# treangenlab/komb

Hardware: AMD Instinct MI355X
Metric: peeled edges/sec (k-truss) (higher is better)
Workload: dtype int32

## Files before the change

### include/komb_accel.h

```cpp
#ifndef KOMB_ACCEL_H
#define KOMB_ACCEL_H

#include <stdint.h>

#ifdef __cplusplus
extern "C" {
#endif

#define KOMB_ACCEL_ABI_VERSION 7

typedef enum komb_status {
    KOMB_OK          =  0,
    KOMB_ERR_ARG     = -1,
    KOMB_ERR_DEVICE  = -2,
    KOMB_ERR_NOMEM   = -3,
    KOMB_ERR_LIMIT   = -4,
    KOMB_ERR_STATE   = -5
} komb_status;

typedef struct komb_ctx komb_ctx;

typedef struct komb_opts {
    int32_t device;
    int32_t verbosity;
// ... 22 lines not shown
    double  ms_compact;
    double  ms_support;
    double  ms_allreduce;
    double  ms_peel;
    double  ms_gather;
    double  ms_corea;
    double  ms_tail;
    int64_t core_local_items, truss_local_items;
    int32_t core_local_units, core_local_sweeps;
    int32_t truss_local_units, truss_local_sweeps;
    double  ms_core_local;
    double  ms_truss_local;
    double  ms_sort;
    int64_t tri_records;
    int32_t index_layout;
    int32_t shard_exchanges;
    double  ms_exchange;
    int64_t exchange_words;
    double  ms_build_h2d;
    double  ms_build_relabel;
    double  ms_prepare;
    int32_t truss_prepared;
    int32_t engine_flags;
    double  ms_prep_vertex;
    double  ms_prep_edges;
    double  ms_prep_rows;
    int32_t stream_retries;
    int32_t reserved0;
} komb_stats;
#define KOMB_ENGINE_LOCAL_FINISH 1
#define KOMB_ENGINE_LDS_TAIL     2
#define KOMB_ENGINE_SHARD_PEEL   4
#define KOMB_ENGINE_TWO_PASS     8

komb_ctx   *komb_create(const komb_opts *opts);
void        komb_destroy(komb_ctx *ctx);
const char *komb_last_error(const komb_ctx *ctx);
int         komb_abi_version(void);
int         komb_set_option(komb_ctx *ctx, const char *name, const char *value);

int komb_graph_from_edges(komb_ctx *ctx, int64_t nv, int64_t n_raw,
                          const int64_t *uv_pairs);

int komb_graph_from_csr(komb_ctx *ctx, int64_t nv, const int64_t *rowptr,
                        const int32_t *col);

int komb_graph_info(komb_ctx *ctx, int64_t *nv, int64_t *ne);

int komb_graph_get_csr(komb_ctx *ctx, int64_t *rowptr, int32_t *col);

int komb_core_run(komb_ctx *ctx);
typedef int (*komb_allreduce_fn)(void *user, void *device_u32, int64_t count);
int komb_core_run_sharded(komb_ctx *ctx, int32_t rank, int32_t world, komb_allreduce_fn allreduce, void *user);
int komb_core_fetch(komb_ctx *ctx, int32_t *degree , int32_t *coreness );
int komb_degree_coreness(komb_ctx *ctx, int32_t *degree, int32_t *coreness);

int komb_onion_run(komb_ctx *ctx);
int komb_onion_fetch(komb_ctx *ctx, int32_t *layer , int32_t *coreness );
int komb_onion_info(komb_ctx *ctx, int64_t *n_layers, int32_t *max_coreness, double *ms);

#define KOMB_COMP_CORE   0
#define KOMB_COMP_TRUSS  1
#define KOMB_COMP_K_MAX (-1)
int komb_components_run(komb_ctx *ctx, int32_t kind, int32_t k);
int komb_components_fetch(komb_ctx *ctx, int32_t *label , int32_t *size );
int komb_components_info(komb_ctx *ctx, int32_t *kind, int32_t *k_used, int64_t *n_members,
// ... 34 lines not shown
```

### komb_amd/api.py

```python
import ctypes
import os

import numpy as np

from . import _lib
from ._lib import KombOpts, KombStats, as_c, ptr


class KombError(RuntimeError):
    def __init__(self, code, msg):
        super().__init__(f"komb_accel error {code}: {msg}")
        self.code = code


def gen_hug_edges(nv, n_cliques, alpha=2.6, seed=42):
    lib = _lib.load()
    n_raw = lib.komb_gen_hug_edges(nv, n_cliques, alpha, seed, None)
    if n_raw < 0:
        raise ValueError("komb_gen_hug_edges: bad arguments")
    uv = np.empty((n_raw, 2), dtype=np.int64)
    got = lib.komb_gen_hug_edges(nv, n_cliques, alpha, seed, ptr(uv))
    assert got == n_raw
    return uv


FORWARD_ENV_OPTIONS = False
OPTION_NAMES = ("FINISH", "LOCAL_LIMIT", "LOCAL_ITEMS", "LOCAL_DENSITY", "LOCAL_DEFER_CHUNKS", "TAIL", "CORE_TAIL", "INDEX",
                "REC_CAP", "OWN_DENSE_CAP", "NO_OWN_DENSE", "NO_REC_SCRATCH", "NO_FIRST_QUEUE", "FULL_CAPS", "PREP_ROW_STAGE", "RETIRE_EVERY", "SHARD_ENGINE",
                "TRI_DEBUG", "POOL_DEBUG", "BUILD_DEBUG", "LOCAL_DEBUG", "TAIL_DEBUG", "COMP_SAMPLE", "POISON")

SENTINEL_I32 = -0x5A5A5A5B


def _out_i32(n):
    return np.full(n, SENTINEL_I32, dtype=np.int32)


def _out_f64(n):
    return np.full(n, np.nan, dtype=np.float64)


class KombAccel:
    def __init__(self, device=0, verbosity=0, flags=0):
        self._lib = _lib.load()
        opts = KombOpts(device=device, verbosity=verbosity)
        opts.reserved[0] = flags
        self._ctx = self._lib.komb_create(ctypes.byref(opts))
        if not self._ctx:
            raise MemoryError("komb_create failed")
        self.device = device
        self.nv = -1
        self.ne = 0
        self._forwarded = {}

    def set_option(self, name, value):
        v = None if value is None else str(value).encode()
        self._check(self._lib.komb_set_option(self._ctx, name.encode(), v))

    def _sync_env_options(self):
        if not FORWARD_ENV_OPTIONS:
            return
# ... 193 lines not shown
```

### komb_amd/csrc/api.cpp

```cpp
#include "common.h"

#include <cerrno>
#include <cmath>
#include <cstdlib>
#include <cstring>
#include <memory>
#include <new>
#include <vector>

using namespace komb;

namespace {

int require_device(komb_ctx *ctx)
{
    if (!ctx) return KOMB_ERR_ARG;
    if (!ctx->device_ok) {
        if (ctx->err.empty()) ctx->err = "no usable HIP device";
        return KOMB_ERR_DEVICE;
    }
    KOMB_HIP(ctx, hipSetDevice(ctx->device));
    ctx->err.clear();
    return KOMB_OK;
}

}

extern "C" {

int komb_abi_version(void) { return KOMB_ACCEL_ABI_VERSION; }

komb_ctx *komb_create(const komb_opts *opts)
{
    komb_ctx *ctx = new (std::nothrow) komb_ctx();
    if (!ctx) return nullptr;
    if (opts) ctx->opts = *opts;
    ctx->device = ctx->opts.device;
    int ndev = 0;
    hipError_t e = hipGetDeviceCount(&ndev);
    if (e != hipSuccess || ndev <= 0) {
        ctx->err = std::string("no usable HIP device: ") + (e != hipSuccess ? hipGetErrorString(e) : "device count is 0");
        (void)hipGetLastError();
        return ctx;
    }
    if (ctx->device < 0 || ctx->device >= ndev) {
        ctx->err = "device ordinal out of range";
        return ctx;
    }
    e = hipSetDevice(ctx->device);
    if (e == hipSuccess) e = hipHostMalloc((void **)&ctx->h_ctrl, 2 * sizeof(PeelCtrl), hipHostMallocDefault);
    if (e == hipSuccess) e = hipHostMalloc((void **)&ctx->h_local, 2 * sizeof(LocalCtrl), hipHostMallocDefault);
    if (e == hipSuccess) e = hipHostMalloc(&ctx->h_stage, kStageBytes, hipHostMallocDefault);
    ctx->stream = nullptr;
    if (e == hipSuccess && !(ctx->opts.reserved[0] & KOMB_CREATE_NULL_STREAM)) { e = hipStreamCreate(&ctx->stream); ctx->own_stream = e == hipSuccess; }
    if (e == hipSuccess && !ctx->timer.init()) e = hipErrorUnknown;
    if (e != hipSuccess) {
        ctx->err = std::string("device initialisation failed: ") + hipGetErrorString(e);
        return ctx;
    }
    ctx->device_ok = true;
    if (!(ctx->opts.reserved[0] & KOMB_CREATE_NO_WARMUP)) warm_up(ctx);
    return ctx;
}

void komb_destroy(komb_ctx *ctx)
{
    if (!ctx) return;
    if (ctx->device_ok) {
        (void)hipSetDevice(ctx->device);
        graph_free(ctx);
        stager_free(ctx);
        ctx->pool.clear();
        ctx->timer.destroy();
        if (ctx->own_stream && ctx->stream) (void)hipStreamDestroy(ctx->stream);
        if (ctx->h_ctrl) (void)hipHostFree(ctx->h_ctrl);
        if (ctx->h_local) (void)hipHostFree(ctx->h_local);
        if (ctx->h_stage) (void)hipHostFree(ctx->h_stage);
    }
    delete ctx;
}

const char *komb_last_error(const komb_ctx *ctx) { return ctx ? ctx->err.c_str() : "null context"; }

int komb_graph_from_edges(komb_ctx *ctx, int64_t nv, int64_t n_raw, const int64_t *uv_pairs)
{
    KOMB_TRY(require_device(ctx));
    return graph_from_edges(ctx, nv, n_raw, uv_pairs);
}

int komb_graph_from_csr(komb_ctx *ctx, int64_t nv, const int64_t *rowptr, const int32_t *col)
{
    KOMB_TRY(require_device(ctx));
    return graph_from_csr(ctx, nv, rowptr, col);
}

int komb_graph_info(komb_ctx *ctx, int64_t *nv, int64_t *ne)
{
    if (!ctx) return KOMB_ERR_ARG;
    if (ctx->nv < 0) KOMB_FAIL(ctx, KOMB_ERR_STATE, "komb_graph_info: no graph loaded");
    if (nv) *nv = ctx->nv;
    if (ne) *ne = ctx->ne;
    return KOMB_OK;
}

int komb_graph_get_csr(komb_ctx *ctx, int64_t *rowptr, int32_t *col)
{
// ... 264 lines not shown
```

### komb_amd/csrc/common.h

```cpp
#pragma once

#include <hip/hip_runtime.h>

#include <chrono>
#include <cstddef>
#include <cstdint>
#include <cstdio>
#include <cstdlib>
#include <cstring>
#include <map>
#include <string>
#include <vector>

#include "komb_accel.h"

#include <roctracer/roctx.h>

namespace komb {

struct Range {
    explicit Range(const char *name) { (void)roctxRangePushA(name); }
    ~Range() { (void)roctxRangePop(); }
    void next(const char *name) { (void)roctxRangePop(); (void)roctxRangePushA(name); }
    Range(const Range &) = delete;
// ... 159 lines not shown
        for (auto &b : blocks) { if (b.used) keep.push_back(b); else (void)hipFree(b.p); }
        blocks.swap(keep);
    }
    void clear()
    {
        for (auto &b : blocks) (void)hipFree(b.p);
        blocks.clear();
    }
};

struct TrussPrep {
    bool valid = false;
    int64_t nv = 0, ne = 0;
    int32_t  *o2i = nullptr, *i2o = nullptr;
    uint32_t *orow = nullptr;
    int32_t  *ocol = nullptr, *osrc = nullptr;
    uint32_t *e2k = nullptr;
    uint4    *vline = nullptr;
    void     *wtasks = nullptr;
    int64_t   n_wtasks = 0;
    int64_t   own_bound = 0;
    double    ms = 0.0;
    double    ms_part[4] = {0, 0, 0, 0};
};

struct komb_ctx {
    komb_opts opts{};
    DevPool pool;
    std::string err;
    bool device_ok = false;
    int device = 0;
    hipStream_t stream = nullptr;
    bool own_stream = false;
    komb::Timer timer;
    std::map<std::string, std::string> options;

    int64_t nv = -1, ne = 0;
    uint32_t *d_o_rowptr = nullptr;
    int32_t  *d_o_col = nullptr;
    TrussPrep prep;

    int32_t *d_deg = nullptr;
    int32_t *d_core = nullptr;
    bool core_done = false;

    int32_t *d_onion_layer = nullptr;
    int32_t *d_onion_core = nullptr;
    int64_t onion_layers = 0;
    int32_t onion_max_core = 0;
    double onion_ms = 0.0;
    bool onion_done = false;

    int32_t *d_comp_label = nullptr;
    int32_t *d_comp_size = nullptr;
    int32_t comp_kind = 0, comp_k = 0;
    int64_t comp_members = 0, comp_count = 0, comp_largest = 0;
    double comp_ms = 0.0;
    bool comp_done = false;

    int64_t t_ne = -1;
    int32_t *d_t_eu = nullptr, *d_t_ev = nullptr, *d_t_truss = nullptr, *d_t_sup = nullptr;
    uint2 *d_t_slice = nullptr;
    uint32_t t_k_lo = 0, t_k_hi = 0;
    bool t_sup_ready = false;
    bool t_own_edges = false;
    int32_t *d_ceu = nullptr, *d_cev = nullptr;
// ... 241 lines not shown
```

### komb_amd/csrc/kcore.hip

```cpp
#include "peel_dev.h"
#include "core_tail.h"
#include "local_dev.h"
#include "shard_dev.h"

#include <cstdlib>

namespace komb {

namespace {

__global__ __launch_bounds__(kBlock) void k_core_init(const uint32_t *__restrict__ rowptr, int64_t nv,
                                                      int32_t *__restrict__ deg, int32_t *__restrict__ degw,
                                                      int32_t *__restrict__ core, uint32_t *__restrict__ init)
{
    uint32_t zeros = 0;
    int32_t lmin = 0x7FFFFFFF;
    for (int64_t v = (int64_t)blockIdx.x * kBlock + threadIdx.x; v < nv; v += (int64_t)gridDim.x * kBlock) {
        const int32_t d = (int32_t)(rowptr[v + 1] - rowptr[v]);
        deg[v] = d; degw[v] = d;
        if (d == 0) { core[v] = 0; ++zeros; }
        else { core[v] = alive_marker((uint32_t)d); lmin = min(lmin, d); }
    }
    block_add_min(zeros, lmin, &init[0], (int32_t *)&init[1]);
}
// ... 242 lines not shown
    peel_ctrl_pre(s, d_grp);
    k_core_init<<<grid_init, kBlock, 0, s>>>(ctx->d_o_rowptr, nv, ctx->d_deg, d_degw, ctx->d_core, d_grp + kInitOff);
    peel_ctrl_init(s, d_ctrl, d_grp, (uint32_t)nv, tail_limit);
    auto run_tail = [&](const int32_t *list, uint32_t n_in) -> int {
        KOMB_HIP(ctx, hipMemsetAsync(T.livebits, 0, live_words * sizeof(unsigned long long), s));
        KOMB_HIP(ctx, hipMemsetAsync(T.cnt, 0, 4 * sizeof(uint32_t), s));
        KOMB_HIP(ctx, hipMemsetAsync(T.rows, 0, (size_t)kCoreTailV * kCoreTailWords * sizeof(unsigned long long), s));
        int64_t gm = ((int64_t)n_in + kBlock - 1) / kBlock;
        k_ctail_mark<<<(int)(gm < 1 ? 1 : (gm > 1024 ? 1024 : gm)), kBlock, 0, s>>>(list, n_in, ctx->d_core, T);
        k_ctail_rows<<<dim3(kCoreTailV, 8), kBlock, 0, s>>>(ctx->d_o_rowptr, ctx->d_o_col, T);
        k_core_tail<false><<<1, 1024, 0, s>>>(d_ctrl, T, d_degw, ctx->d_core, nullptr);
        KOMB_HIP(ctx, d2h(ctx, &ctx->h_ctrl[0], d_ctrl, sizeof(PeelCtrl)));
        return KOMB_OK;
    };
    auto run_local = [&]() -> int {
        const PeelCtrl hc = ctx->h_ctrl[0];
        Range r_local("core: local finish");
        EventSet evs;
        hipEvent_t ev[2] = {nullptr, nullptr};
        for (auto &e : ev) KOMB_HIP(ctx, evs.make(&e));
        (void)hipEventRecord(ev[0], s);
        KOMB_HIP(ctx, hipMemsetAsync(d_livebits, 0, live_words * sizeof(unsigned long long), s));
        LocalStats ls;
        const int rc = local_finish(ctx, bufs, hc, d_ctrl, (uint32_t)nv, ctx->d_core, d_degw, Q.live[hc.live_sel],
            (uint32_t)kWave * CoreLocal::kU, sizeof(uint32_t), local_item_limit(ctx, std::max<uint64_t>(kCoreLocalItems, (uint64_t)ctx->ne / 3)), 0u, false, 0, ctx->d_core,
            [&](const LocalGraph &lg, const int32_t *num, void *items, PeelCtrl *d_cctrl, int32_t launch) {
                CoreCollect C{(uint32_t)nv, ctx->d_o_rowptr, ctx->d_o_col, ctx->d_core, d_livebits, num, lg.off, lg.cur, (uint32_t *)items};
                k_peel_step<CoreCollect><<<grid, kPeelBlock, 0, s>>>(d_cctrl, d_grp, Q, C, launch);
            },
            [&](const LocalGraph &lg, void *items, uint64_t total, LocalCtrl *d_lctrl, uint32_t *d_cnt, int *launches) -> int {
                return local_fixpoint(ctx, d_lctrl, d_cnt, lg, CoreLocal{(const uint32_t *)items}, total, launches);
            },
            &ls,
            [&](const LocalGraph &lg) { k_live_bits<<<(int)((lg.n + 255) / 256 > 1024 ? 1024 : (lg.n + 255) / 256), 256, 0, s>>>(lg.gid, lg.n, d_livebits); });
        (void)hipEventRecord(ev[1], s);
        (void)hipEventSynchronize(ev[1]);
        float ms = 0.f;
        (void)hipEventElapsedTime(&ms, ev[0], ev[1]);
        KOMB_TRY(rc);
        if (ls.refused) { ctx->h_ctrl[0].done = 0; ctx->h_ctrl[0].tail_limit = ls.new_limit; return KOMB_OK; }
        stt.core_local_units = (int32_t)ls.units; stt.core_local_sweeps = ls.sweeps; stt.core_local_items = (int64_t)ls.items;
        stt.ms_core_local = (double)ms;
        PeelCtrl done = hc;
        done.done = 1; done.remaining = 0;
        done.n_levels += (int32_t)ls.levels;
        done.max_level = ls.max_val > done.max_level ? ls.max_val : done.max_level;
        ctx->h_ctrl[0] = done;
        return KOMB_OK;
    };
    int launches = 0, st = KOMB_OK;
    if (sharded) {
        uint32_t iw[2] = {0u, 0u};
        KOMB_HIP(ctx, d2h(ctx, iw, d_grp + kInitOff, sizeof(iw)));
        ShardCore SP{(uint32_t)nv, ctx->d_o_rowptr, ctx->d_o_col, d_degw, ctx->d_core, 0u, 0u};
        shard_bounds((uint64_t)nv, rank, world, &SP.lo, &SP.hi);
        ShardStats ss;
        st = shard_peel(ctx, bufs, SP, d_degw, (uint32_t)nv, iw[0], (int32_t)iw[1], rank, world, fn, user, Q, d_ctrl,
                        [&](int32_t launch) { k_peel_step<ShardCore><<<grid, kPeelBlock, 0, s>>>(d_ctrl, d_grp, Q, SP, launch); },
                        fin == FIN_LOCAL ? tail_limit : 0u, [&]() -> int { return run_local(); }, &ss);
        stt.shard_exchanges = (int32_t)ss.exchanges; stt.ms_exchange = ss.ms_exchange; stt.exchange_words = ss.words;
        launches = ss.launches;
        PeelCtrl fc{};
        fc.done = st == KOMB_OK ? 1 : 2; fc.n_levels = ss.levels; fc.n_rounds = ss.rounds; fc.n_scans = ss.scans; fc.max_level = ss.max_level;
        ctx->h_ctrl[0] = fc;
    } else if (tail_limit && (uint64_t)nv <= tail_limit) {
        st = d2h(ctx, &ctx->h_ctrl[0], d_ctrl, sizeof(PeelCtrl)) == hipSuccess ? KOMB_OK : KOMB_ERR_DEVICE;
        if (st == KOMB_OK && !ctx->h_ctrl[0].done) st = (fin == FIN_LOCAL) ? run_local() : run_tail(nullptr, (uint32_t)nv);
// ... 39 lines not shown
```

### komb_amd/csrc/ktruss.hip

```cpp
#include "peel_dev.h"
#include "truss_tail.h"
#include "local_dev.h"
#include "shard_dev.h"

#include <algorithm>
#include <cstdlib>
#include <cstring>

#include "truss_line.h"
#include "truss_tri.h"
#include "truss_wedge.h"
#include "truss_index.h"
#include "truss_gather.h"

namespace komb {

namespace {

struct TrussProblem {
    static constexpr bool kChain = false;
    static constexpr bool kSingleStep = false;
    uint32_t units;
    const uint2 *off2;
    const int2 *inc;
// ... 224 lines not shown
    if (ctx->t_k_hi < (uint32_t)m) KOMB_HIP(ctx, hipMemsetAsync(ctx->d_t_sup + ctx->t_k_hi, 0, ((size_t)m - ctx->t_k_hi) * sizeof(int32_t), s));
#endif
    k_scatter_len<<<grid_for(m), kBlock, 0, s>>>(ctx->d_t_slice, ctx->prep.e2k, m, ctx->t_k_lo, ctx->t_k_hi, ctx->d_t_sup);
    KOMB_HIP(ctx, hipStreamSynchronize(s));
    ctx->t_sup_ready = true;
    return KOMB_OK;
}

int truss_run(komb_ctx *ctx, const uint8_t *vmask_host, int rank, int world, komb_allreduce_fn fn, void *user)
{
    if (world < 1 || rank < 0 || rank >= world || (world > 1 && !fn))
        KOMB_FAIL(ctx, KOMB_ERR_ARG, "komb_truss_run_sharded: bad rank %d / world %d / callback", rank, world);
    if (ctx->nv < 0) KOMB_FAIL(ctx, KOMB_ERR_STATE, "komb_truss_run: no graph loaded");
    truss_free(ctx);
    hipStream_t s = ctx->stream;
    komb_stats &st = ctx->stats;
    st.triangles = 0; st.truss_levels = st.truss_subrounds = st.truss_launches = 0;
    st.max_trussness = 0; st.ms_support = st.ms_peel = st.ms_orient = st.ms_tri_count = st.ms_tri_fill = st.ms_gather = st.ms_allreduce = st.ms_compact = 0.0;
    st.truss_scans = 0; st.ms_prepare = 0.0; st.truss_prepared = 0; st.ms_prep_vertex = st.ms_prep_edges = st.ms_prep_rows = 0.0;
    auto empty_result = [&]() -> int {
        KOMB_HIP(ctx, ctx->pool.get((void **)&ctx->d_t_eu, 4)); KOMB_HIP(ctx, ctx->pool.get((void **)&ctx->d_t_ev, 4));
        KOMB_HIP(ctx, ctx->pool.get((void **)&ctx->d_t_truss, 4)); KOMB_HIP(ctx, ctx->pool.get((void **)&ctx->d_t_sup, 4));
        ctx->t_own_edges = true; ctx->t_ne = 0; ctx->truss_done = true; ctx->t_sup_ready = true;
        return KOMB_OK;
    };
    if (ctx->nv == 0 || ctx->ne == 0) return empty_result();
    Range r_all("komb_truss_run");
    DevBufs bufs(ctx);

    Range phase("truss: preparation");
    InducedCsr sub;
    TrussPrep sub_prep;
    struct SubGuard { komb_ctx *c; InducedCsr *g; TrussPrep *p; ~SubGuard() { prep_free(c, p); induced_free(c, g); } } sub_guard{ctx, &sub, &sub_prep};
    TrussPrep *tp = &ctx->prep;
    if (vmask_host) {
        ctx->timer.start(s);
        KOMB_TRY(induce_csr(ctx, vmask_host, &sub));
        st.ms_orient = ctx->timer.stop(s);
        if (sub.ns == 0) return empty_result();
        KOMB_TRY(prep_build(ctx, sub.rowptr, sub.col, sub.nv, sub.ns, &sub_prep));
        st.ms_prepare = sub_prep.ms; st.truss_prepared = 1;
        st.ms_prep_vertex = sub_prep.ms_part[0]; st.ms_prep_edges = sub_prep.ms_part[1]; st.ms_prep_rows = sub_prep.ms_part[2];
        tp = &sub_prep;
    } else if (!ctx->prep.valid) {
        KOMB_TRY(prep_ensure(ctx));
        st.ms_prepare = ctx->prep.ms; st.truss_prepared = 1;
        st.ms_prep_vertex = ctx->prep.ms_part[0]; st.ms_prep_edges = ctx->prep.ms_part[1]; st.ms_prep_rows = ctx->prep.ms_part[2];
    }
    const int64_t nv = tp->nv;
    const int64_t m = tp->ne;
    const uint32_t *d_orow = tp->orow;
    const int32_t *d_ocol = tp->ocol;
    const uint4 *d_line = tp->vline;
    const uint2 *d_wtasks = (const uint2 *)tp->wtasks;
    const int64_t n_wtasks = tp->n_wtasks;
    const int gw = grid_for(n_wtasks, kTriWaves);
    phase.next("truss: triangles + incidence index");

    const int ge = grid_for(m);
    const int tri_tv = (int)std::max<int64_t>(1, std::min<int64_t>(kTriV, nv / (256 * KOMB_TRI_EU * kTriWaves * 4)));
    const int64_t ntasks = (nv + tri_tv - 1) / tri_tv;
    const int gt = grid_for(ntasks, kTriWaves);
    uint32_t *d_own = nullptr, *d_other = nullptr, *d_cnt = nullptr, *d_off = nullptr;
    uint2 *d_off2 = nullptr;
    KOMB_HIP(ctx, bufs.alloc(&d_own, 2 * ((size_t)m + 1)));
    d_other = d_own + ((size_t)m + 1);
    KOMB_HIP(ctx, bufs.alloc(&d_cnt, (size_t)m + 1));
    KOMB_HIP(ctx, bufs.alloc(&d_off2, (size_t)m + 4));
    unsigned long long *d_mom = nullptr;
    KOMB_HIP(ctx, bufs.alloc(&d_mom, 12));
    KOMB_HIP(ctx, hipMemsetAsync(d_mom, 0, 12 * sizeof(unsigned long long), s));
    st.ms_allreduce = 0.0;

    const FinishMode fin = finish_mode(ctx, FIN_LOCAL);
    if (fin == FIN_LDS) KOMB_TRY(prep_sources(ctx, tp));
    const int32_t *d_osrc = tp->osrc;
    uint32_t tail_limit = 0;
    if (fin == FIN_LDS) {
        tail_limit = kTailEdges;
        if (const char *tl = ctx_opt(ctx, "TAIL")) tail_limit = (uint32_t)strtoul(tl, nullptr, 10);
        if (tail_limit > kTailMaxEdges) tail_limit = kTailMaxEdges;
    } else if (fin == FIN_LOCAL) tail_limit = local_limit(ctx, (uint64_t)m, 32);
    const bool whole_peel_finish = tail_limit && (uint64_t)m <= tail_limit;
    const bool shard_peel_on = (ctx->shard_peel && world > 1) || ctx_flag(ctx, "SHARD_ENGINE");
    enum { IDX_STREAM = 0, IDX_TWO_PASS = 2 };
    int layout = IDX_STREAM;
    if (const char *ix = ctx_opt(ctx, "INDEX")) {
        if (!strcmp(ix, "two_pass")) layout = IDX_TWO_PASS;
        else if (strcmp(ix, "stream")) KOMB_FAIL(ctx, KOMB_ERR_ARG, "option INDEX=%s: expected stream or two_pass", ix);
    }
    int2 *d_owndense = nullptr;
    unsigned long long *d_ownoff = nullptr, *d_dcur = nullptr;
    uint32_t *d_cnt_ref = nullptr;
    uint32_t *d_toff = nullptr;
    uint32_t *d_grp = nullptr;
    int32_t *d_light0 = nullptr;
    uint32_t *d_bintot = nullptr;
    uint32_t *d_reckey = nullptr;
    int2 *d_recval = nullptr;
    const BinGeom geom = bin_geom(m);
    const int64_t n_bins = (int64_t)geom.nb;
    const TriStream no_stream{nullptr, nullptr, nullptr, 0ull, 0u, 0u, 0};
#ifdef KOMB_DEBUG_SWITCHES
    const int ablate = getenv("KOMB_TRI_ABLATE") ? atoi(getenv("KOMB_TRI_ABLATE")) : 0;
#else
    const int ablate = 0;
#endif
    st.ms_sort = 0.0; st.tri_records = 0; st.ms_compact = 0.0; st.ms_tri_count = 0.0; st.ms_tri_fill = 0.0; st.stream_retries = 0;
    st.index_layout = layout;
    auto zero_counts = [&]() -> hipError_t { return hipMemsetAsync(d_own, 0, 2 * ((size_t)m + 1) * sizeof(uint32_t), s); };
    if (!(world == 1 && layout == IDX_STREAM)) KOMB_HIP(ctx, zero_counts());
    bool have_counts = false;
    if (world > 1) {
        const int64_t task_lo = n_wtasks * rank / world, task_hi = n_wtasks * (rank + 1) / world;
        ctx->timer.start(s);
        k_wedges<TRI_COUNT><<<gw, kBlock, 0, s>>>(d_orow, d_ocol, d_line, d_wtasks, task_lo, task_hi, d_own, d_other, nullptr, nullptr, 0ull, nullptr, no_stream, nullptr, ablate);
// ... 221 lines not shown
        KOMB_HIP(ctx, hipMemsetAsync(T.vmap, 0, (size_t)nv * sizeof(int32_t), s));
        KOMB_HIP(ctx, hipMemsetAsync(T.cnt, 0, 64 * sizeof(uint32_t), s));
        KOMB_HIP(ctx, hipMemsetAsync(T.rows, 0, (size_t)kTailMaxV * kTailRowWords * sizeof(unsigned long long), s));
        const int g = grid_for(n_in, kBlock, 256);
        const bool dbg = ctx_flag(ctx, "TAIL_DEBUG");
        hipEvent_t ev[3] = {nullptr, nullptr, nullptr};
        for (auto &e : ev) (void)hipEventCreate(&e);
        (void)hipEventRecord(ev[0], s);
        k_tail_mark<<<g, kBlock, 0, s>>>(list, n_in, d_sup, d_stamp, d_osrc, d_ocol, T);
        k_tail_number<<<1, kTailMaxV, 0, s>>>(T);
        k_tail_rows<<<g, kBlock, 0, s>>>(list, n_in, d_sup, d_stamp, d_osrc, d_ocol, T);
        (void)hipEventRecord(ev[1], s);
        k_truss_tail<<<1, 1024, 0, s>>>(d_ctrl, T, d_truss);
        (void)hipEventRecord(ev[2], s);
        KOMB_HIP(ctx, d2h(ctx, &ctx->h_ctrl[0], d_ctrl, sizeof(PeelCtrl)));
        ++st.truss_tail_runs;
        float m0 = 0, m1 = 0, m2 = 0;
        (void)hipEventElapsedTime(&m0, ctx->timer.a, ev[0]); (void)hipEventElapsedTime(&m1, ev[0], ev[1]); (void)hipEventElapsedTime(&m2, ev[1], ev[2]);
        for (auto &e : ev) (void)hipEventDestroy(e);
        st.ms_tail += (double)m1 + (double)m2;
        if (dbg) {
            uint32_t h[16];
            KOMB_HIP(ctx, d2h(ctx, h, T.cnt, sizeof(h)));
            fprintf(stderr, "komb tail: %u vertices, %u edges, %s; general engine before it %.1f us, setup %.1f us, tail kernel %.1f us\n",
                    h[0], h[1], ctx->h_ctrl[0].done == 1 ? "done" : "refused", m0 * 1000.f, m1 * 1000.f, m2 * 1000.f);
#ifdef KOMB_TAIL_TIMERS
            fprintf(stderr, "komb tail: us in kernel: load %.1f ranks %.1f supports %.1f scan %.1f mark %.1f triangles %.1f retire %.1f results %.1f\n",
                    h[14] / 100.0, h[15] / 100.0, h[8] / 100.0, h[9] / 100.0, h[10] / 100.0, h[11] / 100.0, h[12] / 100.0, h[13] / 100.0);
#endif
        }
        return KOMB_OK;
    };
    const int gp = peel_grid(m);
    auto run_local = [&]() -> int {
        const PeelCtrl hc = ctx->h_ctrl[0];
        EventSet evs;
        hipEvent_t ev[2] = {nullptr, nullptr};
        for (auto &e : ev) KOMB_HIP(ctx, evs.make(&e));
        (void)hipEventRecord(ev[0], s);
        LocalStats ls;
        const int lrc = local_finish(ctx, bufs, hc, d_ctrl, (uint32_t)m, d_stamp, d_sup, Q.live[hc.live_sel],
            (uint32_t)kWave * TrussLocal::kU, sizeof(uint2), local_item_limit(ctx, kTrussLocalItems), local_density_limit(ctx, kTrussLocalDensity), true, 2, d_truss,
            [&](const LocalGraph &lg, const int32_t *num, void *items, PeelCtrl *d_cctrl, int32_t launch) {
                TrussCollect C{(uint32_t)m, d_off2, d_inc, d_stamp, num, lg.off, lg.cur, (uint2 *)items};
                PeelQueues Qc = Q;
                Qc.rlevel = nullptr;
                k_peel_step<TrussCollect><<<gp, kPeelBlock, 0, s>>>(d_cctrl, d_grp, Qc, C, launch);
            },
            [&](const LocalGraph &lg, void *items, uint64_t total_items, LocalCtrl *d_lctrl, uint32_t *d_cnt, int *nl) -> int {
                return local_fixpoint(ctx, d_lctrl, d_cnt, lg, TrussLocal{(const uint2 *)items}, total_items, nl);
            },
            &ls, [](const LocalGraph &) {});
        (void)hipEventRecord(ev[1], s);
        (void)hipEventSynchronize(ev[1]);
        float ms = 0.f;
        (void)hipEventElapsedTime(&ms, ev[0], ev[1]);
        KOMB_TRY(lrc);
        if (ls.refused) { ctx->h_ctrl[0].done = 0; ctx->h_ctrl[0].tail_limit = ls.new_limit; return KOMB_OK; }
        st.truss_local_units = (int32_t)ls.units; st.truss_local_sweeps = ls.sweeps; st.truss_local_items = (int64_t)ls.items;
        st.ms_truss_local = (double)ms;
        PeelCtrl fin_c = hc;
        fin_c.done = 1; fin_c.remaining = 0;
        fin_c.n_levels += (int32_t)ls.levels;
        fin_c.max_level = ls.max_val > fin_c.max_level ? ls.max_val : fin_c.max_level;
        ctx->h_ctrl[0] = fin_c;
        return KOMB_OK;
    };
    ctx->timer.start(s);
    if (!peel_inited) {
        peel_ctrl_pre(s, d_grp);
        k_peel_init<<<grid_for(m, kBlock, 1024), kBlock, 0, s>>>(m, d_off, d_off2, d_sup, d_stamp, d_st8, d_grp + kInitOff);
    }
    peel_ctrl_init(s, d_ctrl, d_grp, (uint32_t)m, tail_limit);
    int launches = 0, rc = KOMB_OK;
    st.truss_tail_runs = 0; st.ms_tail = 0.0;
    st.truss_local_units = 0; st.truss_local_sweeps = 0; st.truss_local_items = 0; st.ms_truss_local = 0.0;
    st.shard_exchanges = 0; st.ms_exchange = 0.0; st.exchange_words = 0;
    if (shard_peel_on) {
        uint32_t iw[2] = {0u, 0u};
        KOMB_HIP(ctx, d2h(ctx, iw, d_grp + kInitOff, sizeof(iw)));
        ShardTruss SP{(uint32_t)m, d_off2, d_inc, d_sup, d_stamp, 0u, 0u};
        shard_bounds((uint64_t)m, rank, world, &SP.lo, &SP.hi);
        ShardStats ss;
        rc = shard_peel(ctx, bufs, SP, d_sup, (uint32_t)m, iw[0], (int32_t)iw[1], rank, world, fn, user, Q, d_ctrl,
                        [&](int32_t launch) { k_peel_step<ShardTruss><<<gp, kPeelBlock, 0, s>>>(d_ctrl, d_grp, Q, SP, launch); },
// ... 7 lines not shown
        rc = d2h(ctx, &ctx->h_ctrl[0], d_ctrl, sizeof(PeelCtrl)) == hipSuccess ? KOMB_OK : KOMB_ERR_DEVICE;
        if (rc == KOMB_OK && !ctx->h_ctrl[0].done) rc = (fin == FIN_LOCAL) ? run_local() : run_tail(nullptr, (uint32_t)m);
    } else {
        ctx->h_ctrl[0].done = 0;
    }
    for (int guard = 0; rc == KOMB_OK && ctx->h_ctrl[0].done != 1 && ctx->h_ctrl[0].done != 2 && guard < 64; ++guard) {
        if (ctx->h_ctrl[0].done == 3) {
            const PeelCtrl &c = ctx->h_ctrl[0];
            if (fin == FIN_LOCAL) rc = run_local();
            else rc = c.live_mode ? run_tail(Q.live[c.live_sel], c.live_count) : run_tail(nullptr, (uint32_t)m);
            continue;
        }
        int batch = 0;
        rc = drive_peel(ctx, d_ctrl, m, [&](int32_t launch) {
            k_peel_step<TrussProblem><<<gp, kPeelBlock, 0, s>>>(d_ctrl, d_grp, Q, P, launch);
        }, &batch);
        launches += batch;
    }
    st.ms_peel = ctx->timer.stop(s);
    KOMB_TRY(rc);
#ifdef KOMB_STEP_TIMERS
    {
        const PeelCtrl &c = ctx->h_ctrl[0];
        const double n = c.pad1[6] ? (double)c.pad1[6] : 1.0;
        fprintf(stderr, "komb step timers (block 0, %u small multi-workgroup PROCESS steps), us per step: ctrl %.2f queue+slice %.2f items %.2f flush %.2f barrier %.2f ticket %.2f\n",
                c.pad1[6], c.pad1[0] / n / 100.0, c.pad1[1] / n / 100.0, c.pad1[2] / n / 100.0, c.pad1[3] / n / 100.0, c.pad1[4] / n / 100.0, c.pad1[5] / n / 100.0);
    }
#endif
    if (ctx->h_ctrl[0].done != 1) KOMB_FAIL(ctx, KOMB_ERR_DEVICE, "k-truss peel ended in an inconsistent state");
    if (ctx->h_ctrl[0].max_retire_gap > retire_every)
        KOMB_FAIL(ctx, KOMB_ERR_DEVICE, "k-truss peel: %d sub-rounds passed without a RETIRE step (period %d): edge state codes may have wrapped",
                  ctx->h_ctrl[0].max_retire_gap, retire_every);
    st.engine_flags = (layout == IDX_TWO_PASS ? KOMB_ENGINE_TWO_PASS : 0) | (shard_peel_on ? KOMB_ENGINE_SHARD_PEEL : 0) |
                      (st.truss_local_units ? KOMB_ENGINE_LOCAL_FINISH : 0) | (st.truss_tail_runs ? KOMB_ENGINE_LDS_TAIL : 0);
    st.truss_levels = ctx->h_ctrl[0].n_levels;
    st.truss_subrounds = ctx->h_ctrl[0].n_rounds;
    st.truss_launches = launches;
    st.truss_scans = ctx->h_ctrl[0].n_scans;
    st.max_trussness = ctx->h_ctrl[0].max_level + 2;
    for (int i = 0; i < 2; ++i) { bufs.release(Q.light[i]); bufs.release(Q.heavy[i]); bufs.release(Q.live[i]); }
    bufs.release(Q.code);
    bufs.release(d_sup); bufs.release(d_inc);

    phase.next("truss: canonical gather");
    ctx->timer.start(s);
    KOMB_HIP(ctx, ctx->pool.get((void **)&ctx->d_t_truss, (size_t)m * sizeof(int32_t)));
    uint32_t k_lo = 0, k_hi = (uint32_t)m;
    if (!vmask_host) {
        ctx->d_t_eu = ctx->d_ceu; ctx->d_t_ev = ctx->d_cev;
        ctx->t_own_edges = false;
        if (ctx->slice_world > 1) {
            shard_bounds((uint64_t)m, ctx->slice_rank, ctx->slice_world, &k_lo, &k_hi);
#ifndef KOMB_TEST_SKIP_SLICE_ZERO
            if (k_lo) KOMB_HIP(ctx, hipMemsetAsync(ctx->d_t_truss, 0, (size_t)k_lo * sizeof(int32_t), s));
            if (k_hi < (uint32_t)m) KOMB_HIP(ctx, hipMemsetAsync(ctx->d_t_truss + k_hi, 0, ((size_t)m - k_hi) * sizeof(int32_t), s));
#endif
        }
    } else {
        ctx->t_own_edges = true;
        KOMB_HIP(ctx, ctx->pool.get((void **)&ctx->d_t_eu, (size_t)m * sizeof(int32_t)));
        KOMB_HIP(ctx, ctx->pool.get((void **)&ctx->d_t_ev, (size_t)m * sizeof(int32_t)));
        KOMB_TRY(edge_list(ctx, sub.rowptr, sub.col, sub.nv, sub.vold, ctx->d_t_eu, ctx->d_t_ev));
    }
    ctx->t_k_lo = k_lo; ctx->t_k_hi = k_hi;
    k_truss_results<<<grid_for(m), kBlock, 0, s>>>(d_stamp, Q.rlevel, d_truss, tp->e2k, m, k_lo, k_hi, ctx->d_t_truss);
    ctx->d_t_slice = d_off2;
    bufs.detach(d_off2);
    ctx->t_sup_ready = false;
    if (vmask_host) {
        ctx->t_ne = m;
        KOMB_HIP(ctx, ctx->pool.get((void **)&ctx->d_t_sup, (size_t)m * sizeof(int32_t)));
        k_scatter_len<<<grid_for(m), kBlock, 0, s>>>(ctx->d_t_slice, tp->e2k, m, 0u, (uint32_t)m, ctx->d_t_sup);
        ctx->t_sup_ready = true;
    }
    st.ms_gather = ctx->timer.stop(s);
    if (ctx_flag(ctx, "POOL_DEBUG")) {
        size_t held = 0;
        for (const auto &b : ctx->pool.blocks) held += b.bytes;
        fprintf(stderr, "komb pool: %zu blocks, %.2f GB held, %zu hipMalloc calls so far (%.1f ms inside them), %zu trims\n", ctx->pool.blocks.size(), held / 1e9, ctx->pool.n_malloc, ctx->pool.ms_malloc, ctx->pool.n_trim);
    }
    if (vmask_host) KOMB_HIP(ctx, hipStreamSynchronize(s));
    ctx->t_ne = m;
    ctx->truss_done = true;
    return KOMB_OK;
}

}
```

### komb_amd/csrc/local_dev.h

```cpp
#pragma once

#include "peel_dev.h"

namespace komb {

constexpr int kLocBlock = 512;
constexpr int kLocWaves = kLocBlock / kWave;
constexpr int kLocHB = 4096;
constexpr int kLocBins = kLocHB / kLocBlock;
constexpr int kCntWays = 8;
constexpr int kCntWords = (5 * kCntWays + 5) * 32;
constexpr int kCntTimerWords = 6 * 12 * 2;
constexpr int kHvU = 8;
constexpr uint32_t kKeyBins = 4096;
constexpr uint32_t kMedMax = 2048;
constexpr int kGiantWin = 8;
constexpr uint32_t kGiantChunk = 8192;
constexpr int kLocBatch = 6;


struct LocalGraph {
    uint32_t n, nh;
    uint32_t *off;
    int32_t *val;
// ... 699 lines not shown
    hipError_t e = hipStreamSynchronize(s);
    if (per_sweep) {
        fprintf(stderr, "komb local sweeps (us):");
        for (size_t i = 1; i < sw.size(); ++i) { float ms = 0.f; (void)hipEventElapsedTime(&ms, sw[i - 1], sw[i]); fprintf(stderr, " %.0f", ms * 1e3f); }
        fprintf(stderr, "\n");
    }
    if (launches_out) *launches_out = launches;
    if (status != KOMB_OK || e != hipSuccess)
        KOMB_FAIL(ctx, KOMB_ERR_DEVICE, "local fixed point: HIP failure (%s)", hipGetErrorString(e));
    if (stuck) KOMB_FAIL(ctx, KOMB_ERR_DEVICE, "local fixed point: the sweeps make no progress (sweep %d)", (int)seen_iters);
    return KOMB_OK;
}

static __global__ __launch_bounds__(kBlock) void k_local_zero(uint32_t *a, uint32_t na, uint32_t *b, uint32_t nb, uint32_t *c, uint32_t nc,
                                                       uint32_t *d, uint32_t nd, uint32_t *e, uint32_t ne)
{
    const uint32_t t = blockIdx.x * kBlock + threadIdx.x, step = gridDim.x * kBlock;
    for (uint32_t i = t; i < na; i += step) a[i] = 0u;
    for (uint32_t i = t; i < nb; i += step) b[i] = 0u;
    for (uint32_t i = t; i < nc; i += step) c[i] = 0u;
    for (uint32_t i = t; i < nd; i += step) d[i] = 0u;
    for (uint32_t i = t; i < ne; i += step) e[i] = 0u;
}

struct LocalStats {
    uint32_t units = 0, heavy = 0, levels = 0;
    int32_t max_val = 0;
    int sweeps = 0, launches = 0;
    uint64_t items = 0, evals = 0;
    bool refused = false;
    uint32_t new_limit = 0;
};

template <class LaunchCollect, class RunFix, class AfterNumber>
int local_finish(komb_ctx *ctx, DevBufs &bufs, const PeelCtrl &hc, PeelCtrl *d_ctrl, uint32_t units, const int32_t *marker,
                 const int32_t *key, const int32_t *live_list, uint32_t light_max, size_t item_bytes, uint64_t item_limit, uint32_t max_density, bool use_list, int32_t add, int32_t *out,
                 LaunchCollect &&launch_collect, RunFix &&run_fix, LocalStats *ls, AfterNumber &&after_number)
{
    hipStream_t s = ctx->stream;
    const uint32_t n = hc.remaining;
    if (n == 0) KOMB_FAIL(ctx, KOMB_ERR_STATE, "local finish: nothing left to hand over");
    const bool dbg = ctx_opt(ctx, "LOCAL_DEBUG") != nullptr;
    EventSet evs;
    hipEvent_t ev[5] = {nullptr, nullptr, nullptr, nullptr, nullptr};
    if (dbg) for (auto &e : ev) (void)evs.make(&e);
    auto stamp = [&](int i) { if (dbg) (void)hipEventRecord(ev[i], s); };
    stamp(0);
    const int32_t *list = hc.live_mode ? live_list : nullptr;
    const uint32_t n_in = hc.live_mode ? hc.live_count : units;
    LocalGraph g{};
    int32_t *d_num = nullptr;
    LocalCtrl *d_lctrl = nullptr;
    PeelCtrl *d_cctrl = nullptr;
    uint32_t *d_present = nullptr;
    const size_t present_words = ((size_t)units >> 5) + 2 > kFinWords ? ((size_t)units >> 5) + 2 : (size_t)kFinWords;
    KOMB_HIP(ctx, bufs.alloc(&d_num, (size_t)units));
    KOMB_HIP(ctx, bufs.alloc(&g.off, (size_t)n + 1));
    KOMB_HIP(ctx, bufs.alloc(&g.len, (size_t)n + 1));
    KOMB_HIP(ctx, bufs.alloc(&g.val, (size_t)n));
    KOMB_HIP(ctx, bufs.alloc(&g.mark[0], (size_t)n));
    KOMB_HIP(ctx, bufs.alloc(&g.mark[1], (size_t)n));
    KOMB_HIP(ctx, bufs.alloc(&g.gid, (size_t)n));
    KOMB_HIP(ctx, bufs.alloc(&g.cur, (size_t)n));
    KOMB_HIP(ctx, bufs.alloc(&g.list, (size_t)n));
    KOMB_HIP(ctx, bufs.alloc(&g.giant, (size_t)n));
    KOMB_HIP(ctx, bufs.alloc(&g.khist, (size_t)kKeyBins));
    KOMB_HIP(ctx, bufs.alloc(&d_lctrl, 1));
    uint32_t *d_cnt = nullptr;
    KOMB_HIP(ctx, bufs.alloc(&d_cnt, (size_t)kCntWords + kCntTimerWords));
    KOMB_HIP(ctx, bufs.alloc(&d_cctrl, 1));
// ... 54 lines not shown
    if (g.ng) {
        KOMB_HIP(ctx, bufs.alloc(&g.gchunk, (size_t)g.nchunk));
        KOMB_HIP(ctx, bufs.alloc(&g.gacc, (size_t)g.ng));
        KOMB_HIP(ctx, bufs.alloc(&g.gwin, (size_t)g.ng * kGiantWin));
        KOMB_HIP(ctx, bufs.alloc(&g.gnote, (size_t)g.ng));
        k_local_chunks<<<(int)(g.ng > 1024u ? 1024u : g.ng), kBlock, 0, s>>>(g);
    }
    int32_t K = 0x7FFFFFFF;
    {
        uint64_t ge = 0;
        for (int32_t k = (int32_t)kKeyBins - 1; k >= 0; --k) {
            ge += kh[(size_t)k];
            if (ge >= (uint64_t)k) { if (k < (int32_t)kKeyBins - 1) K = k; break; }
        }
    }
    stamp(1);
    after_number(g);
    KOMB_HIP(ctx, bufs.alloc((unsigned char **)&d_items, (size_t)total * item_bytes));

    peel_collect_ctrl(s, d_cctrl, d_ctrl);
    PeelCtrl hcc{};
    int32_t cl = 1;
    for (int guard = 0; guard < 16 && hcc.done == 0; ++guard) {
        for (int i = 0; i < 3; ++i) launch_collect(g, d_num, d_items, d_cctrl, cl++);
        KOMB_HIP(ctx, d2h(ctx, &hcc, d_cctrl, sizeof(PeelCtrl)));
        cl = hcc.seq;
    }
    if (hcc.done != 1) KOMB_FAIL(ctx, KOMB_ERR_DEVICE, "local finish: collect pass did not complete (state %d)", hcc.done);
    int64_t gn = ((int64_t)n + kBlock - 1) / kBlock;
    const int grid_n = (int)(gn > 1024 ? 1024 : gn);
    k_local_check<<<grid_n, kBlock, 0, s>>>(g, d_lctrl);
    if (K != 0x7FFFFFFF) k_local_clamp<<<grid_n, kBlock, 0, s>>>(g, K);
    stamp(2);

    int launches = 0;
    KOMB_TRY(run_fix(g, d_items, (uint64_t)total, d_lctrl, d_cnt, &launches));
    stamp(3);
    k_local_finish<<<grid_n, kBlock, 0, s>>>(g, add, out, d_present, d_lctrl);
    k_local_levels<<<(int)(present_words / kBlock + 1 > 256 ? 256 : present_words / kBlock + 1), kBlock, 0, s>>>(d_present, (uint32_t)present_words, d_cnt, d_lctrl);
    stamp(4);
    KOMB_HIP(ctx, d2h(ctx, &hl, d_lctrl, sizeof(LocalCtrl)));
    if (dbg) {
        float t[4] = {0, 0, 0, 0};
        for (int i = 0; i < 4; ++i) (void)hipEventElapsedTime(&t[i], ev[i], ev[i + 1]);
        fprintf(stderr, "komb local finish: %u units (%u heavy, %u of them long; bound %d), %u items; number+scan %.1f us, collect %.1f us, %d sweeps (%d launches, %u evaluations) %.1f us, scatter %.1f us\n",
                n, g.nh, g.ng, K == 0x7FFFFFFF ? -1 : K, total, t[0] * 1e3f, t[1] * 1e3f, hl.iters, launches, hl.evals, t[2] * 1e3f, t[3] * 1e3f);
    }
#ifdef KOMB_LOCAL_TIMERS
    {
        unsigned long long tm[72];
        KOMB_HIP(ctx, d2h(ctx, tm, d_cnt + kCntWords, sizeof(tm)));
        for (int sw = 0; sw < 6; ++sw) {
            const unsigned long long *t = tm + sw * 12;
            const double nwv = t[10] ? (double)t[10] : 1.0;
            fprintf(stderr, "komb local timers, sweep %d (%llu waves), us per wave: hscan %.1f medium %.1f workgroup %.1f setup %.1f load+count %.1f search %.1f notify %.1f; "
                            "batches/wave %.2f groups/wave %.2f; slowest wave %.1f us\n",
                    sw == 0 ? 1 : sw * 4, t[10], t[0] / nwv / 100.0, t[1] / nwv / 100.0, t[2] / nwv / 100.0, t[3] / nwv / 100.0, t[4] / nwv / 100.0, t[5] / nwv / 100.0,
                    t[6] / nwv / 100.0, t[7] / nwv, t[8] / nwv, t[9] / 100.0);
        }
    }
#endif
    if (hl.bad) KOMB_FAIL(ctx, KOMB_ERR_DEVICE, "local finish: %u consistency failures in the compact index", hl.bad);
    if (!hl.done) KOMB_FAIL(ctx, KOMB_ERR_DEVICE, "local finish: launch budget exhausted before the fixed point");
    if (ls) {
        ls->units = n; ls->heavy = g.nh; ls->levels = hl.levels; ls->max_val = hl.max_val;
        ls->sweeps = hl.iters; ls->launches = launches; ls->items = total; ls->evals = hl.evals;
    }
    release_all();
    return KOMB_OK;
}

}
```

### komb_amd/csrc/truss_gather.h

```cpp
#pragma once

#include "peel_dev.h"

namespace komb {

namespace {

__global__ __launch_bounds__(kBlock) void k_truss_results(const int32_t *__restrict__ stamp, const int32_t *__restrict__ rlevel,
                                                         const int32_t *__restrict__ truss,
                                                         const uint32_t *__restrict__ e2k, int64_t m, uint32_t k_lo, uint32_t k_hi,
                                                         int32_t *__restrict__ tr_out)
{
    for (int64_t e = (int64_t)blockIdx.x * kBlock + threadIdx.x; e < m; e += (int64_t)gridDim.x * kBlock) {
        const int32_t s = stamp[e];
        const int32_t t = marker_alive(s) ? truss[e] : rlevel[s] + 2;
        const uint32_t k = e2k[e];
        if (k - k_lo < k_hi - k_lo) tr_out[k] = t;
    }
}

__global__ __launch_bounds__(kBlock) void k_scatter_len(const uint2 *__restrict__ off2, const uint32_t *__restrict__ e2k, int64_t m,
                                                       uint32_t k_lo, uint32_t k_hi, int32_t *__restrict__ out)
{
    for (int64_t e = (int64_t)blockIdx.x * kBlock + threadIdx.x; e < m; e += (int64_t)gridDim.x * kBlock) {
        const uint32_t k = e2k[e];
        if (k - k_lo < k_hi - k_lo) out[k] = (int32_t)off2[e].y;
    }
}

}

}
```

Before: 4.076 billion.

## Overlap truss result gather with local finish on a low-priority side stream

Splits the final trussness gather into an early pass over already-peeled edges, launched on a new low-priority side stream right after the local-finish collect step, and a late pass over only the locally finished edges, run on the main stream after the finish. The aim is to hide the full-edge gather behind the local fixpoint sweeps and shrink the serial tail. This adds a second stream, events and cross-stream waits, and the side kernel may compete with the fixpoint kernels for compute units. It is only active when the local finish path with a tail limit is used.

```diff
diff --git a/include/komb_accel.h b/include/komb_accel.h
--- a/include/komb_accel.h
+++ b/include/komb_accel.h
@@ -78,6 +78,7 @@
 #define KOMB_ENGINE_LDS_TAIL     2
 #define KOMB_ENGINE_SHARD_PEEL   4
 #define KOMB_ENGINE_TWO_PASS     8
+#define KOMB_ENGINE_RESULTS_OVERLAP 16
 
 komb_ctx   *komb_create(const komb_opts *opts);
 void        komb_destroy(komb_ctx *ctx);
diff --git a/komb_amd/api.py b/komb_amd/api.py
--- a/komb_amd/api.py
+++ b/komb_amd/api.py
@@ -27,6 +27,7 @@
 FORWARD_ENV_OPTIONS = False
 OPTION_NAMES = ("FINISH", "LOCAL_LIMIT", "LOCAL_ITEMS", "LOCAL_DENSITY", "LOCAL_DEFER_CHUNKS", "TAIL", "CORE_TAIL", "INDEX",
                 "REC_CAP", "OWN_DENSE_CAP", "NO_OWN_DENSE", "NO_REC_SCRATCH", "NO_FIRST_QUEUE", "FULL_CAPS", "PREP_ROW_STAGE", "RETIRE_EVERY", "SHARD_ENGINE",
+                "RESULTS_OVERLAP", "RESULTS_GRID",
                 "TRI_DEBUG", "POOL_DEBUG", "BUILD_DEBUG", "LOCAL_DEBUG", "TAIL_DEBUG", "COMP_SAMPLE", "POISON")
 
 SENTINEL_I32 = -0x5A5A5A5B
diff --git a/komb_amd/csrc/api.cpp b/komb_amd/csrc/api.cpp
--- a/komb_amd/csrc/api.cpp
+++ b/komb_amd/csrc/api.cpp
@@ -53,6 +53,11 @@
     if (e == hipSuccess) e = hipHostMalloc(&ctx->h_stage, kStageBytes, hipHostMallocDefault);
     ctx->stream = nullptr;
     if (e == hipSuccess && !(ctx->opts.reserved[0] & KOMB_CREATE_NULL_STREAM)) { e = hipStreamCreate(&ctx->stream); ctx->own_stream = e == hipSuccess; }
+    if (e == hipSuccess && ctx->own_stream) {
+        int least = 0, greatest = 0;
+        if (hipDeviceGetStreamPriorityRange(&least, &greatest) != hipSuccess) { (void)hipGetLastError(); least = 0; }
+        e = hipStreamCreateWithPriority(&ctx->side, hipStreamDefault, least);
+    }
     if (e == hipSuccess && !ctx->timer.init()) e = hipErrorUnknown;
     if (e != hipSuccess) {
         ctx->err = std::string("device initialisation failed: ") + hipGetErrorString(e);
@@ -72,6 +77,7 @@
         stager_free(ctx);
         ctx->pool.clear();
         ctx->timer.destroy();
+        if (ctx->side) (void)hipStreamDestroy(ctx->side);
         if (ctx->own_stream && ctx->stream) (void)hipStreamDestroy(ctx->stream);
         if (ctx->h_ctrl) (void)hipHostFree(ctx->h_ctrl);
         if (ctx->h_local) (void)hipHostFree(ctx->h_local);
diff --git a/komb_amd/csrc/common.h b/komb_amd/csrc/common.h
--- a/komb_amd/csrc/common.h
+++ b/komb_amd/csrc/common.h
@@ -215,6 +215,7 @@
     int device = 0;
     hipStream_t stream = nullptr;
     bool own_stream = false;
+    hipStream_t side = nullptr;
     komb::Timer timer;
     std::map<std::string, std::string> options;
 
diff --git a/komb_amd/csrc/kcore.hip b/komb_amd/csrc/kcore.hip
--- a/komb_amd/csrc/kcore.hip
+++ b/komb_amd/csrc/kcore.hip
@@ -298,7 +298,8 @@
                 return local_fixpoint(ctx, d_lctrl, d_cnt, lg, CoreLocal{(const uint32_t *)items}, total, launches);
             },
             &ls,
-            [&](const LocalGraph &lg) { k_live_bits<<<(int)((lg.n + 255) / 256 > 1024 ? 1024 : (lg.n + 255) / 256), 256, 0, s>>>(lg.gid, lg.n, d_livebits); });
+            [&](const LocalGraph &lg) { k_live_bits<<<(int)((lg.n + 255) / 256 > 1024 ? 1024 : (lg.n + 255) / 256), 256, 0, s>>>(lg.gid, lg.n, d_livebits); },
+            [](const LocalGraph &) {}, [](const LocalGraph &) {});
         (void)hipEventRecord(ev[1], s);
         (void)hipEventSynchronize(ev[1]);
         float ms = 0.f;
diff --git a/komb_amd/csrc/ktruss.hip b/komb_amd/csrc/ktruss.hip
--- a/komb_amd/csrc/ktruss.hip
+++ b/komb_amd/csrc/ktruss.hip
@@ -280,6 +280,8 @@
     InducedCsr sub;
     TrussPrep sub_prep;
     struct SubGuard { komb_ctx *c; InducedCsr *g; TrussPrep *p; ~SubGuard() { prep_free(c, p); induced_free(c, g); } } sub_guard{ctx, &sub, &sub_prep};
+    EventSet side_ev;
+    struct SidePass { hipStream_t side; bool in_flight; ~SidePass() { if (in_flight) (void)hipStreamSynchronize(side); } } side_pass{ctx->side, false};
     TrussPrep *tp = &ctx->prep;
     if (vmask_host) {
         ctx->timer.start(s);
@@ -330,6 +332,8 @@
         if (tail_limit > kTailMaxEdges) tail_limit = kTailMaxEdges;
     } else if (fin == FIN_LOCAL) tail_limit = local_limit(ctx, (uint64_t)m, 32);
     const bool whole_peel_finish = tail_limit && (uint64_t)m <= tail_limit;
+    const char *ro = ctx_opt(ctx, "RESULTS_OVERLAP");
+    const bool overlap_on = ctx->side && fin == FIN_LOCAL && tail_limit && !(ro && !strcmp(ro, "0"));
     const bool shard_peel_on = (ctx->shard_peel && world > 1) || ctx_flag(ctx, "SHARD_ENGINE");
     enum { IDX_STREAM = 0, IDX_TWO_PASS = 2 };
     int layout = IDX_STREAM;
@@ -617,6 +621,46 @@
         return KOMB_OK;
     };
     const int gp = peel_grid(m);
+    uint32_t k_lo = 0, k_hi = (uint32_t)m;
+    bool results_ready = false;
+    auto results_setup = [&]() -> int {
+        if (results_ready) return KOMB_OK;
+        KOMB_HIP(ctx, ctx->pool.get((void **)&ctx->d_t_truss, (size_t)m * sizeof(int32_t)));
+        if (!vmask_host && ctx->slice_world > 1) {
+            shard_bounds((uint64_t)m, ctx->slice_rank, ctx->slice_world, &k_lo, &k_hi);
+#ifndef KOMB_TEST_SKIP_SLICE_ZERO
+            if (k_lo) KOMB_HIP(ctx, hipMemsetAsync(ctx->d_t_truss, 0, (size_t)k_lo * sizeof(int32_t), s));
+            if (k_hi < (uint32_t)m) KOMB_HIP(ctx, hipMemsetAsync(ctx->d_t_truss + k_hi, 0, ((size_t)m - k_hi) * sizeof(int32_t), s));
+#endif
+        }
+        results_ready = true;
+        return KOMB_OK;
+    };
+    hipEvent_t rev[5] = {nullptr, nullptr, nullptr, nullptr, nullptr};
+    if (overlap_on) {
+        KOMB_HIP(ctx, side_ev.make(&rev[0], hipEventDisableTiming));
+        for (int i = 1; i < 5; ++i) KOMB_HIP(ctx, side_ev.make(&rev[i]));
+    }
+    bool early_ran = false, late_ran = false;
+    int early_grid = std::max(1, grid_for(m) / 4);
+    if (const char *rg = ctx_opt(ctx, "RESULTS_GRID")) early_grid = std::max(1, std::min(atoi(rg), 256 * 16));
+    auto results_early = [&](const LocalGraph &) {
+        if (!overlap_on || early_ran) return;
+        if (results_setup() != KOMB_OK) return;
+        if (hipEventRecord(rev[0], s) != hipSuccess || hipStreamWaitEvent(ctx->side, rev[0], 0) != hipSuccess) { (void)hipGetLastError(); return; }
+        (void)hipEventRecord(rev[1], ctx->side);
+        side_pass.in_flight = true;
+        k_truss_results_early<<<early_grid, kBlock, 0, ctx->side>>>(d_stamp, Q.rlevel, tp->e2k, m, k_lo, k_hi, ctx->d_t_truss);
+        (void)hipEventRecord(rev[2], ctx->side);
+        early_ran = true;
+    };
+    auto results_late = [&](const LocalGraph &lg) {
+        if (!early_ran || late_ran) return;
+        (void)hipEventRecord(rev[3], s);
+        k_truss_results_late<<<grid_for(lg.n), kBlock, 0, s>>>(lg.gid, lg.n, (uint32_t)m, d_truss, tp->e2k, k_lo, k_hi, ctx->d_t_truss);
+        (void)hipEventRecord(rev[4], s);
+        late_ran = true;
+    };
     auto run_local = [&]() -> int {
         const PeelCtrl hc = ctx->h_ctrl[0];
         EventSet evs;
@@ -635,7 +679,7 @@
             [&](const LocalGraph &lg, void *items, uint64_t total_items, LocalCtrl *d_lctrl, uint32_t *d_cnt, int *nl) -> int {
                 return local_fixpoint(ctx, d_lctrl, d_cnt, lg, TrussLocal{(const uint2 *)items}, total_items, nl);
             },
-            &ls, [](const LocalGraph &) {});
+            &ls, [](const LocalGraph &) {}, results_early, results_late);
         (void)hipEventRecord(ev[1], s);
         (void)hipEventSynchronize(ev[1]);
         float ms = 0.f;
@@ -709,7 +753,8 @@
         KOMB_FAIL(ctx, KOMB_ERR_DEVICE, "k-truss peel: %d sub-rounds passed without a RETIRE step (period %d): edge state codes may have wrapped",
                   ctx->h_ctrl[0].max_retire_gap, retire_every);
     st.engine_flags = (layout == IDX_TWO_PASS ? KOMB_ENGINE_TWO_PASS : 0) | (shard_peel_on ? KOMB_ENGINE_SHARD_PEEL : 0) |
-                      (st.truss_local_units ? KOMB_ENGINE_LOCAL_FINISH : 0) | (st.truss_tail_runs ? KOMB_ENGINE_LDS_TAIL : 0);
+                      (st.truss_local_units ? KOMB_ENGINE_LOCAL_FINISH : 0) | (st.truss_tail_runs ? KOMB_ENGINE_LDS_TAIL : 0) |
+                      (early_ran ? KOMB_ENGINE_RESULTS_OVERLAP : 0);
     st.truss_levels = ctx->h_ctrl[0].n_levels;
     st.truss_subrounds = ctx->h_ctrl[0].n_rounds;
     st.truss_launches = launches;
@@ -721,18 +766,11 @@
 
     phase.next("truss: canonical gather");
     ctx->timer.start(s);
-    KOMB_HIP(ctx, ctx->pool.get((void **)&ctx->d_t_truss, (size_t)m * sizeof(int32_t)));
-    uint32_t k_lo = 0, k_hi = (uint32_t)m;
+    if (early_ran && !late_ran) KOMB_FAIL(ctx, KOMB_ERR_DEVICE, "k-truss results: the early pass ran without the late one");
+    KOMB_TRY(results_setup());
     if (!vmask_host) {
         ctx->d_t_eu = ctx->d_ceu; ctx->d_t_ev = ctx->d_cev;
         ctx->t_own_edges = false;
-        if (ctx->slice_world > 1) {
-            shard_bounds((uint64_t)m, ctx->slice_rank, ctx->slice_world, &k_lo, &k_hi);
-#ifndef KOMB_TEST_SKIP_SLICE_ZERO
-            if (k_lo) KOMB_HIP(ctx, hipMemsetAsync(ctx->d_t_truss, 0, (size_t)k_lo * sizeof(int32_t), s));
-            if (k_hi < (uint32_t)m) KOMB_HIP(ctx, hipMemsetAsync(ctx->d_t_truss + k_hi, 0, ((size_t)m - k_hi) * sizeof(int32_t), s));
-#endif
-        }
     } else {
         ctx->t_own_edges = true;
         KOMB_HIP(ctx, ctx->pool.get((void **)&ctx->d_t_eu, (size_t)m * sizeof(int32_t)));
@@ -740,7 +778,8 @@
         KOMB_TRY(edge_list(ctx, sub.rowptr, sub.col, sub.nv, sub.vold, ctx->d_t_eu, ctx->d_t_ev));
     }
     ctx->t_k_lo = k_lo; ctx->t_k_hi = k_hi;
-    k_truss_results<<<grid_for(m), kBlock, 0, s>>>(d_stamp, Q.rlevel, d_truss, tp->e2k, m, k_lo, k_hi, ctx->d_t_truss);
+    if (early_ran) KOMB_HIP(ctx, hipStreamWaitEvent(s, rev[2], 0));
+    else k_truss_results<<<grid_for(m), kBlock, 0, s>>>(d_stamp, Q.rlevel, d_truss, tp->e2k, m, k_lo, k_hi, ctx->d_t_truss);
     ctx->d_t_slice = d_off2;
     bufs.detach(d_off2);
     ctx->t_sup_ready = false;
@@ -751,6 +790,12 @@
         ctx->t_sup_ready = true;
     }
     st.ms_gather = ctx->timer.stop(s);
+    if (early_ran) {
+        side_pass.in_flight = false;
+        float ms_early = 0.f, ms_late = 0.f;
+        (void)hipEventElapsedTime(&ms_early, rev[1], rev[2]); (void)hipEventElapsedTime(&ms_late, rev[3], rev[4]);
+        st.ms_gather += (double)ms_early + (double)ms_late;
+    }
     if (ctx_flag(ctx, "POOL_DEBUG")) {
         size_t held = 0;
         for (const auto &b : ctx->pool.blocks) held += b.bytes;
diff --git a/komb_amd/csrc/local_dev.h b/komb_amd/csrc/local_dev.h
--- a/komb_amd/csrc/local_dev.h
+++ b/komb_amd/csrc/local_dev.h
@@ -755,10 +755,11 @@
     uint32_t new_limit = 0;
 };
 
-template <class LaunchCollect, class RunFix, class AfterNumber>
+template <class LaunchCollect, class RunFix, class AfterNumber, class AfterCollect, class AfterFinish>
 int local_finish(komb_ctx *ctx, DevBufs &bufs, const PeelCtrl &hc, PeelCtrl *d_ctrl, uint32_t units, const int32_t *marker,
                  const int32_t *key, const int32_t *live_list, uint32_t light_max, size_t item_bytes, uint64_t item_limit, uint32_t max_density, bool use_list, int32_t add, int32_t *out,
-                 LaunchCollect &&launch_collect, RunFix &&run_fix, LocalStats *ls, AfterNumber &&after_number)
+                 LaunchCollect &&launch_collect, RunFix &&run_fix, LocalStats *ls, AfterNumber &&after_number, AfterCollect &&after_collect,
+                 AfterFinish &&after_finish)
 {
     hipStream_t s = ctx->stream;
     const uint32_t n = hc.remaining;
@@ -879,6 +880,7 @@
     k_local_check<<<grid_n, kBlock, 0, s>>>(g, d_lctrl);
     if (K != 0x7FFFFFFF) k_local_clamp<<<grid_n, kBlock, 0, s>>>(g, K);
     stamp(2);
+    after_collect(g);
 
     int launches = 0;
     KOMB_TRY(run_fix(g, d_items, (uint64_t)total, d_lctrl, d_cnt, &launches));
@@ -886,6 +888,7 @@
     k_local_finish<<<grid_n, kBlock, 0, s>>>(g, add, out, d_present, d_lctrl);
     k_local_levels<<<(int)(present_words / kBlock + 1 > 256 ? 256 : present_words / kBlock + 1), kBlock, 0, s>>>(d_present, (uint32_t)present_words, d_cnt, d_lctrl);
     stamp(4);
+    after_finish(g);
     KOMB_HIP(ctx, d2h(ctx, &hl, d_lctrl, sizeof(LocalCtrl)));
     if (dbg) {
         float t[4] = {0, 0, 0, 0};
diff --git a/komb_amd/csrc/truss_gather.h b/komb_amd/csrc/truss_gather.h
--- a/komb_amd/csrc/truss_gather.h
+++ b/komb_amd/csrc/truss_gather.h
@@ -19,6 +19,29 @@
     }
 }
 
+__global__ __launch_bounds__(kBlock) void k_truss_results_early(const int32_t *__restrict__ stamp, const int32_t *__restrict__ rlevel,
+                                                               const uint32_t *__restrict__ e2k, int64_t m, uint32_t k_lo, uint32_t k_hi,
+                                                               int32_t *__restrict__ tr_out)
+{
+    for (int64_t e = (int64_t)blockIdx.x * kBlock + threadIdx.x; e < m; e += (int64_t)gridDim.x * kBlock) {
+        const int32_t s = stamp[e];
+        if (marker_alive(s)) continue;
+        const uint32_t k = e2k[e];
+        if (k - k_lo < k_hi - k_lo) tr_out[k] = rlevel[s] + 2;
+    }
+}
+__global__ __launch_bounds__(kBlock) void k_truss_results_late(const int32_t *__restrict__ gid, uint32_t n, uint32_t m, const int32_t *__restrict__ truss,
+                                                              const uint32_t *__restrict__ e2k, uint32_t k_lo, uint32_t k_hi,
+                                                              int32_t *__restrict__ tr_out)
+{
+    for (uint32_t i = blockIdx.x * kBlock + threadIdx.x; i < n; i += gridDim.x * kBlock) {
+        const uint32_t e = (uint32_t)gid[i];
+        if (e >= m) continue;
+        const uint32_t k = e2k[e];
+        if (k - k_lo < k_hi - k_lo) tr_out[k] = truss[e];
+    }
+}
+
 __global__ __launch_bounds__(kBlock) void k_scatter_len(const uint2 *__restrict__ off2, const uint32_t *__restrict__ e2k, int64_t m,
                                                        uint32_t k_lo, uint32_t k_hi, int32_t *__restrict__ out)
 {
```

Measured after the change: 4.097 billion (median of 3 runs). Within noise of the previous version (+0.5%).
